# aouyang1/go-muse

Measured on AMD Instinct MI355X. Metric: series-pairs XCorr/sec at N=4096, 1M-series batch; achieved HBM GB/s, higher is better.
Workload: dtype f64

## Files before the change

### go-muse_amd/binding.py

```python
import ctypes
import os

import numpy as np

from . import build as _build

_i32 = ctypes.c_int32
_i64 = ctypes.c_int64
_f64 = ctypes.c_double
_vp = ctypes.c_void_p
_dp = ctypes.POINTER(ctypes.c_double)
_i32p = ctypes.POINTER(ctypes.c_int32)
_i64p = ctypes.POINTER(ctypes.c_int64)

MUSE_OK = 0
MUSE_ERR_INVALID = -1
MUSE_ERR_LENGTH = -2
MUSE_ERR_ZERO_STD = -3
MUSE_ERR_NO_DEVICE = -4
MUSE_ERR_HIP = -5
MUSE_ERR_UNSUPPORTED = -6
MUSE_ERR_NOMEM = -7
MUSE_ERR_EMPTY = -8
MUSE_LAG_WINDOW_MAX = 63
# ... 118 lines not shown
    "muse_batch_score_many_in_window": (ctypes.c_int, [ctypes.POINTER(_vp), _i32, _i32]),
    "muse_batch_run_many_in_window": (ctypes.c_int, [ctypes.POINTER(_vp), _i32, _i32p, _i32, _i32, _i32, _f64, _i32, _i32,
                                                     _i64p, _i32p, _dp, _i32p, _dp]),
    "muse_test_many_in_window_plan": (ctypes.c_int, [_i32, _i32, _i32, _i32, _i32p]),
    "muse_batch_score_many_in_lag_range": (ctypes.c_int, [ctypes.POINTER(_vp), _i32, _i32, _i32]),
    "muse_batch_run_many_in_lag_range": (ctypes.c_int, [ctypes.POINTER(_vp), _i32, _i32p, _i32, _i32, _i32, _i32, _f64, _i32, _i32,
                                                        _i64p, _i32p, _dp, _i32p, _dp]),
    "muse_test_many_lag_range_plan": (ctypes.c_int, [_i32, _i32, _i32, _i32, _i32, _i32p]),
    "muse_test_window_many_plan_rows": (ctypes.c_int, [_i32, _i32, _i32p, _i32p, _i32p, _i32p, _i32p, _i32p]),
    "muse_batch_run_many": (ctypes.c_int, [ctypes.POINTER(_vp), _i32, _i32p, _i32, _i32, _i32, _f64, _i32, _i32,
                                           _i64p, _i32p, _dp, _i32p, _dp]),
    "muse_batch_free": (ctypes.c_int, [_vp]),
    "muse_xcorr_with_x": (ctypes.c_int, [_vp, _dp, _dp, _i32, _i32, _dp, _i32p, _dp, _i32p]),
    "muse_xcorr": (ctypes.c_int, [_vp, _dp, _i32, _dp, _i32, _i32, _i32, _dp, _i32p, _dp, _i32p]),
    "muse_xcorr_groups": (ctypes.c_int, [_vp, _vp, _i32, _i32, _i32p, _dp, _i32p, _dp]),
    "muse_xcorr_batch": (ctypes.c_int, [_vp, _dp, _dp, _i64, _i32, _i32, _i32, _i32, _i32p, _dp, _i32p, _dp]),
    "muse_ctx_set_spectrum_cache": (ctypes.c_int, [_vp, _i32]),
    "muse_group_spectrum_cache": (ctypes.c_int, [_vp, _i64p, _i64p]),
    "muse_group_drop_spectrum_cache": (ctypes.c_int, [_vp]),
    "muse_test_spectrum_cache_limits": (ctypes.c_int, [_vp, _i64, _i64]),
    "muse_test_spectrum_cache_reader": (ctypes.c_int, [_vp, _i32]),
    "muse_test_spectrum_cache_policy": (ctypes.c_int, [_i64, _i32, _i32, _i32, _i64, _i64, _i64, _i32p, _i64p, _i64p]),
    "muse_test_batch_redo_pairs": (ctypes.c_int, [_vp, _i64p, _i64, _i64p]),
    "muse_next_pow2": (_i64, [_f64]),
}


class MuseError(RuntimeError):
    def __init__(self, status, message):
        super().__init__("muse_hip status %d: %s" % (status, message))
        self.status = status
        self.message = message


_lib = None


def lib_path():
    return _build.LIB


def load():
    global _lib
    if _lib is None:
        path = lib_path()
        if not os.path.exists(path):
# ... 36 lines not shown
```

### go-muse_amd/csrc/capi_batch.hip

```cpp
#include "capi_internal.h"
#include "xcorr_huge.h"

using namespace muse;


int ilog2(int64_t n)
{
    int l = 0;
    while (((int64_t)1 << l) < n)
        l++;
    return l;
}

int build_spectrum(muse_ctx *ctx, const double *ref_host, int N, int n, int normalize, double x_scale,
                          double xc_scale, double2 *X, double2 *xc, float2 *xcf, double *xs, int *zero_std)
{
    double *dref = nullptr;
    int *dstat = nullptr;
    double2 *dscr = nullptr;
    HIP_TRY(dmalloc(ctx, &dref, (size_t)N * sizeof(double)));
    hipError_t e = dmalloc(ctx, &dstat, sizeof(int));
    if (e == hipSuccess && n > GENERIC_LDS_MAX_N)
        e = dmalloc(ctx, &dscr, (size_t)n * sizeof(double2));
    if (e == hipSuccess)
// ... 518 lines not shown
    return MUSE_OK;
}

extern "C" int muse_test_batch_redo_pairs(muse_batch *b, int64_t *pairs, int64_t cap, int64_t *count)
{
    if (!b || !count || cap < 0 || (cap > 0 && !pairs))
        return fail(MUSE_ERR_INVALID, "bad redo-list arguments");
    *count = 0;
    int rc = use_device(b->ctx);
    if (rc)
        return rc;
    HIP_TRY(hipStreamSynchronize(b->stream()));
    if (!b->ovf_count || !b->ovf_list.p)
        return MUSE_OK;
    int listed = 0;
    HIP_TRY(hipMemcpy(&listed, b->ovf_count, sizeof(int), hipMemcpyDeviceToHost));
    *count = listed;
    const int64_t k = std::min<int64_t>(std::min<int64_t>(listed, cap), b->ovf_list.cap);
    if (k > 0)
        HIP_TRY(hipMemcpy(pairs, b->ovf_list.p, (size_t)k * sizeof(long long), hipMemcpyDeviceToHost));
    return MUSE_OK;
}

extern "C" int muse_batch_score(muse_batch *b)
{
    return batch_score(b, ScorePass{});
}

static int check_mask(const muse_batch *b, int variant, const LagRange &mask)
{
    if (!(variant == KERNEL_R16_FOLD || variant == KERNEL_R16_OCC3 || (variant == KERNEL_SMALL && b->logn <= 11)) || 2 * mask.hi > b->n)
        return fail(MUSE_ERR_UNSUPPORTED, "the masked transform pass runs on the default kernels of FFT lengths 512 ... 4096");
    if (2 * mask.lneg > b->n - 2)
        return fail(MUSE_ERR_UNSUPPORTED, "the masked transform pass takes at most n / 2 - 1 lags below zero");
    return MUSE_OK;
}

int batch_score_check(muse_batch *b, const LagRange *mask, int *variant)
{
    *variant = -1;
    if (b->n > GENERIC_MAX_N)
        return b->g->f32 ? fail(MUSE_ERR_UNSUPPORTED, "float32-storage groups run on the default kernels only (FFT lengths 512 ... 16384)") : MUSE_OK;
    const KernelChoice kc = choose_kernel(b, (b->g->M + 1) / 2);
    if (kc.error)
        return fail(MUSE_ERR_UNSUPPORTED, "%s", kc.error);
    if (mask && check_mask(b, kc.variant, *mask))
// ... 47 lines not shown
        rc = check_mask(b, variant, *mask);
        if (rc)
            return rc;
        b->origin = ScoreOrigin::in_window(MUSE_IN_WINDOW_MASKED, *mask, variant);
        set_window(p, *mask);
    }
    const bool allow_spectrum_cache = pass.allow_spectrum_cache;
    const SlideFuse *slide = pass.slide;
    if (slide) {
        if (variant != KERNEL_R16_FOLD || allow_spectrum_cache)
            return fail(MUSE_ERR_INVALID, "the fused slide runs in the default n = 4096 kernel, off the rows");
        p.slide_tails = slide->tails;
        p.slide_k = slide->k;
    }
    if (variant == KERNEL_GENERIC && b->n <= GENERIC_LDS_MAX_N)
        p.gscratch = nullptr;
    LaunchTimer timer(ctx, false, st);
    LaunchTimer redo_timer(ctx, true, st);
    if (variant == KERNEL_R16_FOLD) {
        HIP_TRY(b->ovf_list.ensure(ctx, 2 * p.npairs, st));
        p.ovf_count = b->ovf_count;
        p.work_counter = b->ovf_count + 1;
        p.ovf_list = b->ovf_list.p;
        HIP_TRY(hipMemsetAsync(b->ovf_count, 0, 2 * sizeof(int), st));
        ZcPlan plan;
        std::unique_lock<std::mutex> zc_lock(b->g->ready_mu, std::defer_lock);
        if (allow_spectrum_cache && !mask && spectrum_cache_candidate(b, variant)) {
            zc_lock.lock();
            rc = plan_spectrum_cache(b, plan);
            if (rc)
                return rc;
            if (!plan.use)
                zc_lock.unlock();
        }
        HIP_TRY(timer.begin());
        if (plan.use) {
            bool launched = false;
            const auto next_launch = [&]() {
                const hipError_t e = launched ? hipMemsetAsync(b->ovf_count + 1, 0, sizeof(int), st) : hipSuccess;
                launched = true;
                return e;
            };
            const bool occ4_reader = ctx->zc_reader.load() == 1;
            for (const auto &sg : plan.readers) {
                FusedParams r = p;
                r.npairs = sg.pairs;
                HIP_TRY(next_launch());
                HIP_TRY(launch_cached(r, SpectrumCacheArgs{sg.zc(), sg.zstat(), sg.pair0, sg.pairs}, ctx->num_cus, st, occ4_reader));
            }
            if (plan.tail_pair0 < p.npairs) {
                FusedParams w = p;
                w.npairs = p.npairs - plan.tail_pair0;
                HIP_TRY(next_launch());
                HIP_TRY(launch_cache_fill(w, SpectrumCacheArgs{plan.tail_zpairs ? plan.tail_seg.zc() : nullptr,
                                                               plan.tail_zpairs ? plan.tail_seg.zstat() : nullptr,
                                                               plan.tail_pair0, plan.tail_zpairs}, ctx->num_cus, st));
            }
            zc_lock.unlock();
        } else {
            HIP_TRY(launch_fused(p, variant, ctx->num_cus, st));
        }
        HIP_TRY(timer.end());
        FusedParams q = p;
        q.slide_tails = nullptr;
        q.slide_k = 0;
        q.pair_list = b->ovf_list.p;
        q.pair_count = b->ovf_count;
        q.dense_total = ctx->variant == 0 ? p.npairs : 0;
        q.npairs = std::min<long long>(p.npairs, (long long)ctx->num_cus * 3);
        HIP_TRY(redo_timer.begin());
        HIP_TRY(launch_fused(q, KERNEL_R16_OCC3, ctx->num_cus, st));
        HIP_TRY(redo_timer.end());
        if (p.npairs >= 1024 && !(b->handoff_host && b->handoff_M == M && b->handoff_rewrites == b->g->rewrites)) {
            if (!b->handoff_host)
                HIP_TRY(hmalloc(ctx, &b->handoff_host, sizeof(int)));
            *b->handoff_host = 0;
            b->handoff_M = M;
            b->handoff_rewrites = b->g->rewrites;
            HIP_TRY(hipMemcpyAsync(b->handoff_host, b->ovf_count, sizeof(int), hipMemcpyDeviceToHost, st));
        }
    } else if (variant == KERNEL_LONG) {
        HIP_TRY(b->ovf_list.ensure(ctx, 2 * p.npairs, st));
        p.ovf_count = b->ovf_count;
        p.ovf_list = b->ovf_list.p;
        HIP_TRY(hipMemsetAsync(b->ovf_count, 0, 2 * sizeof(int), st));
        HIP_TRY(timer.begin());
        HIP_TRY(launch_fused(p, variant, ctx->num_cus, st));
        HIP_TRY(timer.end());
        FusedParams q = p;
        q.pair_list = b->ovf_list.p;
        q.pair_count = b->ovf_count;
        q.npairs = std::min<long long>(p.npairs, (long long)ctx->num_cus * STOCKHAM_GLOBAL_WGS_PER_CU);
        HIP_TRY(redo_timer.begin());
        HIP_TRY(launch_fused(q, KERNEL_STOCKHAM, ctx->num_cus, st));
        HIP_TRY(redo_timer.end());
    } else {
        HIP_TRY(timer.begin());
        HIP_TRY(launch_fused(p, variant, ctx->num_cus, st));
        HIP_TRY(timer.end());
    }
    return MUSE_OK;
}

extern "C" int muse_batch_scores(muse_batch *b, int32_t *lag, double *mv)
{
    int rc = muse_batch_score(b);
    if (rc)
        return rc;
    const int64_t M = b->g->M;
    if (M == 0)
        return MUSE_OK;
    if (!lag || !mv)
        return fail(MUSE_ERR_INVALID, "NULL output");
    HIP_TRY(hipMemcpyAsync(lag, b->lag.p, (size_t)M * sizeof(int), hipMemcpyDeviceToHost, b->stream()));
    HIP_TRY(hipMemcpyAsync(mv, b->mv.p, (size_t)M * sizeof(double), hipMemcpyDeviceToHost, b->stream()));
    HIP_TRY(hipStreamSynchronize(b->stream()));
    return MUSE_OK;
}

extern "C" int muse_batch_kernel_name(muse_batch *b, char *name, int32_t cap)
{
    if (!b || !name || cap < 1)
        return fail(MUSE_ERR_INVALID, "NULL argument");
    char k[96] = "xcorr_fused_generic";
    const char *padded = b->N < b->n ? "true" : "false", *f32 = b->g->f32 ? "true" : "false";
    const ScoreOrigin &o = b->origin;
    if (o.slide == MUSE_SLIDE_IN_WINDOW_FUSED) {
        snprintf(k, sizeof(k), "xcorr_fused_n4096_fold<false, %s, %s, %s, true>", padded, f32, o.kind == ScoreOrigin::MASKED ? "true" : "false");
    } else if (o.kind == ScoreOrigin::MASKED) {
        if (o.variant == ScoreOrigin::MANY && b->n == 4096)
            snprintf(k, sizeof(k), "xcorr_fused_n4096_fold_multi<%s, %s, true>", padded, f32);
        else if (o.variant == ScoreOrigin::MANY)
            snprintf(k, sizeof(k), "xcorr_fused_small<%d, %s, true, false, true>", b->logn, padded);
        else if (b->n == 4096 && o.variant == KERNEL_R16_OCC3)
            snprintf(k, sizeof(k), "xcorr_fused_n4096_occ4<%s, 3, false, %s, true>", padded, f32);
        else if (b->n == 4096)
            snprintf(k, sizeof(k), "xcorr_fused_n4096_fold<false, %s, %s, true>", padded, f32);
        else
            snprintf(k, sizeof(k), "xcorr_fused_small<%d, %s, false, %s, true>", b->logn, padded, f32);
// ... 99 lines not shown
```

### go-muse_amd/csrc/capi_context.hip

```cpp
#include "capi_internal.h"

using namespace muse;


thread_local std::string g_last_error;

int fail(int status, const char *fmt, ...)
{
    char buf[512];
    va_list ap;
    va_start(ap, fmt);
    vsnprintf(buf, sizeof(buf), fmt, ap);
    va_end(ap);
    g_last_error = buf;
    return status;
}

extern "C" int muse_abi_version(void) { return MUSE_HIP_ABI_VERSION; }
extern "C" const char *muse_last_error(void) { return g_last_error.c_str(); }
extern "C" const char *muse_status_string(int s)
{
    switch (s) {
    case MUSE_OK: return "ok";
    case MUSE_ERR_INVALID: return "invalid argument";
// ... 286 lines not shown
                            fprintf(f, " %llu", h[((size_t)wg * 16 + w) * 16 + i]);
                        fprintf(f, "\n");
                    }
                fclose(f);
            }
        }
    }
#endif
    (void)hipFree(ctx->dbg_stamps);
    rows_slots_free(ctx);
    huge_free(ctx);
    ctx->gscratch.release(ctx);
    ctx->zscratch.release(ctx);
    ctx->many_tab.release(ctx);
    for (auto &p : ctx->small_free)
        (void)hipHostFree(p.first);
    ctx->small_free.clear();
    pool_drain(ctx);
    for (auto *ev : {&ctx->events, &ctx->redo_events})
        for (auto &e : *ev) {
            (void)hipEventDestroy(e.first);
            (void)hipEventDestroy(e.second);
        }
    (void)hipFree(ctx->tw1);
    (void)hipFree(ctx->tw2);
    (void)hipFree(ctx->twm);
    (void)hipFree(ctx->twmf);
    (void)hipFree(ctx->tw1f);
    (void)hipFree(ctx->g2);
    (void)hipFree(ctx->g3a);
    (void)hipFree(ctx->g3b);
    for (int k = 0; k < 5; k++)
        (void)hipFree(ctx->gsmall[k]);
    (void)hipFree(ctx->wsplit);
    for (int k = 0; k < 3; k++)
        (void)hipFree(ctx->twl[k]);
    for (double *b : ctx->stage_pool)
        (void)hipHostFree(b);
    (void)hipFree(ctx->tw2f);
    if (ctx->probe_stream) {
        if (ctx->probe_buf)
            *((volatile int *)(ctx->probe_buf + 2 * PROBE_WINDOWS) + 1) = 1;
        (void)hipStreamSynchronize(ctx->probe_stream);
        (void)hipStreamDestroy(ctx->probe_stream);
    }
    if (ctx->probe_buf)
// ... 11 lines not shown

extern "C" int muse_ctx_synchronize(muse_ctx *ctx)
{
    int rc = use_device(ctx);
    if (rc)
        return rc;
    HIP_TRY(hipStreamSynchronize(ctx->stream));
    return MUSE_OK;
}

extern "C" int muse_ctx_trim(muse_ctx *ctx)
{
    int rc = use_device(ctx);
    if (rc)
        return rc;
    pool_drain(ctx);
    std::vector<std::pair<unsigned char *, int>> slots;
    {
        std::lock_guard<std::mutex> lock(ctx->small_mu);
        slots.swap(ctx->small_free);
    }
    for (auto &p : slots)
        (void)hipHostFree(p.first);
    return MUSE_OK;
}

extern "C" int muse_test_pool_stats(muse_ctx *ctx, int64_t *dev_idle_bytes, int64_t *dev_idle_blocks, int64_t *host_idle_bytes,
                                    int64_t *host_idle_blocks)
{
    if (!ctx)
        return fail(MUSE_ERR_INVALID, "NULL context");
    {
        std::lock_guard<std::mutex> lock(ctx->dev_pool.mu);
        if (dev_idle_bytes)
            *dev_idle_bytes = (int64_t)ctx->dev_pool.idle_bytes;
        if (dev_idle_blocks)
            *dev_idle_blocks = (int64_t)ctx->dev_pool.idle.size();
    }
    {
        std::lock_guard<std::mutex> lock(ctx->host_pool.mu);
        if (host_idle_bytes)
            *host_idle_bytes = (int64_t)ctx->host_pool.idle_bytes;
        if (host_idle_blocks)
            *host_idle_blocks = (int64_t)ctx->host_pool.idle.size();
    }
    return MUSE_OK;
// ... 25 lines not shown
    if (!ctx || !(variant == 0 || variant == 1 || variant == 7 || variant == 10 || variant == 11 || variant == 12 || variant == 13 || variant == 14 || variant == 15))
        return fail(MUSE_ERR_INVALID, "bad kernel variant (0 auto, 1 generic, 7 rescaling n=4096, 10 default n=4096, 11 Stockham, 12 half-round, 13 long series, 14 real transform, 15 real transform on the 16 x 1024 split)");
    ctx->variant = variant;
    return MUSE_OK;
}

extern "C" int muse_ctx_set_screening(muse_ctx *ctx, int32_t enable)
{
    if (!ctx)
        return fail(MUSE_ERR_INVALID, "NULL context");
    ctx->screening = enable != 0;
    ctx->screen_min_rows = enable > 1 ? enable : 0;
    return MUSE_OK;
}

extern "C" int muse_ctx_kernel_timing(muse_ctx *ctx, int32_t enable)
{
    if (!ctx)
        return fail(MUSE_ERR_INVALID, "NULL context");
    ctx->timing = enable != 0;
    return MUSE_OK;
}

static int drain_events(std::vector<std::pair<hipEvent_t, hipEvent_t>> &ev, double &ms_sum, int64_t &count)
{
    for (auto &e : ev) {
        HIP_TRY(hipEventSynchronize(e.second));
        float ms = 0.f;
        HIP_TRY(hipEventElapsedTime(&ms, e.first, e.second));
        ms_sum += (double)ms;
        count += 1;
        (void)hipEventDestroy(e.first);
        (void)hipEventDestroy(e.second);
    }
    ev.clear();
    return MUSE_OK;
}

extern "C" int muse_ctx_kernel_time(muse_ctx *ctx, double *total_ms, int64_t *launches)
{
    int rc = use_device(ctx);
    if (rc)
        return rc;
    rc = drain_events(ctx->events, ctx->total_ms, ctx->launches);
    if (rc)
        return rc;
    if (total_ms)
        *total_ms = ctx->total_ms;
    if (launches)
        *launches = ctx->launches;
    ctx->total_ms = 0.0;
    ctx->launches = 0;
    return MUSE_OK;
}

extern "C" int muse_ctx_redo_time(muse_ctx *ctx, double *total_ms, int64_t *brackets)
{
    int rc = use_device(ctx);
    if (rc)
        return rc;
    rc = drain_events(ctx->redo_events, ctx->redo_ms, ctx->redo_launches);
    if (rc)
        return rc;
    if (total_ms)
        *total_ms = ctx->redo_ms;
    if (brackets)
        *brackets = ctx->redo_launches;
    ctx->redo_ms = 0.0;
    ctx->redo_launches = 0;
    return MUSE_OK;
}

extern "C" int muse_ctx_device_pci_bus_id(muse_ctx *ctx, char *out, int32_t cap)
{
    if (!ctx || !out || cap < 16)
        return fail(MUSE_ERR_INVALID, "muse_ctx_device_pci_bus_id: NULL argument or a buffer under 16 bytes");
    snprintf(out, (size_t)cap, "%s", ctx->pci);
    return MUSE_OK;
}

extern "C" int muse_test_clock_probe_stop(muse_ctx *ctx)
{
    if (!ctx)
        return fail(MUSE_ERR_INVALID, "NULL context");
// ... 72 lines not shown
```

### go-muse_amd/csrc/capi_internal.h

```cpp
#pragma once
#include <hip/hip_runtime.h>

#include <algorithm>
#include <atomic>
#include <mutex>
#include <cmath>
#include <cstdarg>
#include <cstdio>
#include <cstdlib>
#include <cstring>
#include <ctime>
#include <limits>
#include <map>
#include <new>
#include <string>
#include <unordered_map>
#include <utility>
#include <vector>

#include "muse_hip.h"
#include "muse_hip_test.h"
#include "xcorr_kernels.h"

using namespace muse;
// ... 35 lines not shown
        if (e == hipSuccess)
            cap = count;
        return e;
    }
    void release(muse_ctx *ctx)
    {
        pool_free(ctx, Host, p);
        p = nullptr;
        cap = 0;
    }
};
template <class T> using HostBuf = PoolBuf<T, true>;
struct HugeWork {
    double2 *thi[4] = {nullptr, nullptr, nullptr, nullptr}, *tlo[4] = {nullptr, nullptr, nullptr, nullptr};
    PoolBuf<double2> Y, T;
    PoolBuf<double> part, snorm, sfin, sfin_x, amax;
    PoolBuf<double2> Y2;
    PoolBuf<double> amax2;
    hipStream_t stream2 = nullptr;
    hipEvent_t fork = nullptr, join = nullptr;
};
constexpr int64_t ZC_MIN_ROWS = 65536;
constexpr int ZC_MAX_SEGMENTS = 64;
constexpr int PROBE_WINDOWS = 4096;
struct muse_ctx {
    int device = 0;
    hipStream_t stream = nullptr;
    hipStream_t copy_stream = nullptr;
    int num_cus = 0;
    int64_t hbm = 0;
    char name[64] = {0};
    double2 *tw1 = nullptr, *tw2 = nullptr, *twm = nullptr;
    double2 *g2 = nullptr, *g3a = nullptr, *g3b = nullptr;
    double2 *twl[3] = {nullptr, nullptr, nullptr};
    double2 *gsmall[5] = {nullptr, nullptr, nullptr, nullptr, nullptr};
    double2 *wsplit = nullptr;
    float2 *tw1f = nullptr, *tw2f = nullptr, *twmf = nullptr;
    PoolBuf<double2> gscratch;
    std::vector<double *> stage_pool;
    std::mutex stage_mu;
    PoolBuf<double2> zscratch;
    PoolBuf<void *> many_tab;
    std::vector<void *> many_host;
    double screen_delta = 1e-4;
    int screening = 0;
    int64_t screen_min_rows = 0;
    double screen_e_scale = 1.0;
    int variant = 0;
    int xcorr_repeat = 1;
    unsigned long long *dbg_stamps = nullptr;
    hipStream_t probe_stream = nullptr;
    unsigned long long *probe_buf = nullptr;
    bool timing = false;
    std::vector<std::pair<hipEvent_t, hipEvent_t>> events, redo_events;
    double total_ms = 0.0, redo_ms = 0.0;
    int64_t launches = 0, redo_launches = 0;
    char pci[32] = {0};
    MemPool dev_pool, host_pool;
    HugeWork huge;
    int huge_batch_mb = 0;
    std::mutex huge_mu;
    std::mutex small_mu;
    std::vector<std::pair<unsigned char *, int>> small_free;
    unsigned long long small_token = 0;
    std::mutex timing_mu;
    std::atomic<bool> rows_always_copy{false};
    std::vector<void *> rows_slots;
    std::mutex rows_mu;
    std::atomic<int> zc_mode{1};
    std::atomic<int64_t> zc_min_rows{ZC_MIN_ROWS};
    std::atomic<int64_t> zc_budget{-1};
    std::atomic<int> zc_reader{0};
    std::atomic<int> win_rows_slices{0};
    std::atomic<bool> in_window_force{false};
    std::atomic<int> slide_in_window_force{0};
    std::atomic<bool> gather_nt{false};
    std::atomic<int> refs{1};
// ... 25 lines not shown
    hipEvent_t uploaded = nullptr;
    bool upload_pending = false;
    std::mutex ready_mu;
    HostBuf<long long> gidx_host;
    PoolBuf<long long> gidx_dev;
    hipEvent_t gather_done = nullptr;
    HostBuf<unsigned char> slide_host;
    PoolBuf<unsigned char> slide_dev;
    hipEvent_t slide_copied[2] = {nullptr, nullptr};
    struct ZcSegment {
        void *mem = nullptr;
        int64_t pair0 = 0, pairs = 0;
        double2 *zc() const { return (double2 *)mem; }
        double *zstat() const { return (double *)((char *)mem + (size_t)pairs * 4096 * sizeof(double2)); }
    };
    enum { ZC_NONE = 0, ZC_DECLINED = 1, ZC_VALID = 2 };
    std::vector<ZcSegment> zc_segs;
    int zc_state = ZC_NONE;
    int64_t zc_rows = 0, zc_bytes = 0;
    uint64_t zc_rewrites = 0;
    int64_t zc_passes = 0;
    int64_t zc_declined_M = -1;
    bool transient = false;
};

inline std::atomic<uint64_t> g_spectrum_serial{0};
struct muse_spectrum {
    std::atomic<int> refs{1};
    const uint64_t serial = g_spectrum_serial.fetch_add(1, std::memory_order_relaxed) + 1;
    double2 *X = nullptr, *xc = nullptr, *xcp = nullptr;
    double2 *xcw = nullptr;
    float2 *xcf = nullptr;
    double *xs = nullptr;
    double *c1 = nullptr;
    double xmax = -1.0;
};

inline int window_lneg(int L, int n) { return 2 * L == n ? L - 1 : L; }
struct LagRange {
    int hi, lneg, origin;
    int rows() const { return origin + hi + 1; }
    bool every_lag(int64_t n) const { return 2 * (int64_t)hi == n && lneg == n / 2 - 1; }
};
inline LagRange lag_window_range(int64_t n, int64_t L)
{
    const int hi = (int)std::min<int64_t>(L, n / 2);
// ... 22 lines not shown
    static ScoreOrigin packed(int32_t tiles) { return ScoreOrigin{PACKED, LagRange{0, 0, 0}, 0, tiles}; }
    static ScoreOrigin in_window(int32_t path, const LagRange &w, int32_t variant = 0) { return ScoreOrigin{(Kind)path, w, variant}; }
    int32_t in_window_path() const { return kind > OWN ? (int32_t)kind : 0; }
    int32_t mfma_tiles() const { return (window.rows() + 15) / 16; }
};

struct muse_batch {
    muse_ctx *ctx = nullptr;
    muse_group *g = nullptr;
    hipStream_t own_stream = nullptr;
    hipStream_t stream() const { return own_stream ? own_stream : ctx->stream; }
    int32_t N = 0, n = 0, logn = 0;
    muse_spectrum *sp = nullptr;
    double *c1 = nullptr;
    double2 *X = nullptr, *xc = nullptr;
    double2 *xcp = nullptr;
    double2 *xcw = nullptr;
    float2 *xcf = nullptr;
    double *xs = nullptr;
    int *ovf_count = nullptr;
    int *handoff_host = nullptr;
    int64_t handoff_M = -1;
    uint64_t handoff_rewrites = 0;
    PoolBuf<long long> ovf_list;
    PoolBuf<double> mv;
    PoolBuf<int> lag;
    unsigned char *small_out = nullptr;
    int small_cap = 0;
    PoolBuf<int> gid_dev;
    std::vector<int32_t> gid_host;
    bool gid_valid = false;
    PoolBuf<unsigned long long> gkey;
    PoolBuf<long long> gfirst, gwin;
    GroupWork gw() const { return GroupWork{gkey.p, gfirst.p, gwin.p}; }
    PoolBuf<muse_record> rec;
    PoolBuf<unsigned long long> selkey;
    PoolBuf<muse_record> cand;
    PoolBuf<int> cnt;
    HostBuf<muse_record> cand_host;
    HostBuf<int> cnt_host;
    HostBuf<muse_record> rec_host;
    HostBuf<unsigned long long> key_host;
    PoolBuf<unsigned> scr_flags;
    PoolBuf<double> scr_var;
    PoolBuf<unsigned char> include;
    PoolBuf<unsigned long long> scr_keys;
// ... 21 lines not shown
    int64_t guard_trips = 0;
    uint64_t guard_salt = 0;
    int32_t lag_window = -1;
    int32_t win_key = -1;
    PoolBuf<double> win_e, win_pw;
    bool windowed() const { return lag_window >= 0; }
    ScoreOrigin origin;
};

int use_device(muse_ctx *ctx);

struct LaunchTimer {
    muse_ctx *ctx;
    hipEvent_t e0 = nullptr, e1 = nullptr;
    bool redo;
    hipStream_t stream;
    explicit LaunchTimer(muse_ctx *c, bool redo_ = false, hipStream_t s = nullptr) : ctx(c), redo(redo_), stream(s ? s : c->stream) {}
    LaunchTimer(const LaunchTimer &) = delete;
    LaunchTimer &operator=(const LaunchTimer &) = delete;
    hipError_t begin()
    {
        if (!ctx->timing)
            return hipSuccess;
        hipError_t e = hipEventCreate(&e0);
        if (e == hipSuccess)
            e = hipEventCreate(&e1);
        if (e == hipSuccess)
            e = hipEventRecord(e0, stream);
        return e;
    }
    hipError_t end()
    {
        if (!e0 || !e1)
            return hipSuccess;
        const hipError_t e = hipEventRecord(e1, stream);
        if (e == hipSuccess) {
            std::lock_guard<std::mutex> lock(ctx->timing_mu);
            (redo ? ctx->redo_events : ctx->events).emplace_back(e0, e1);
            e0 = e1 = nullptr;
        }
        return e;
    }
    ~LaunchTimer()
    {
        if (e0)
            (void)hipEventDestroy(e0);
        if (e1)
            (void)hipEventDestroy(e1);
// ... 24 lines not shown
void adopt_spectrum(muse_batch *b);
int build_spectrum(muse_ctx *ctx, const double *ref_host, int N, int n, int normalize, double x_scale,
                          double xc_scale, double2 *X, double2 *xc, float2 *xcf, double *xs, int *zero_std);
hipError_t ensure_gscratch(muse_ctx *ctx, int64_t n, int slices_per_cu = muse::GSCRATCH_SLICES_PER_CU);
hipError_t ensure_twl(muse_ctx *ctx, int64_t n);
int ensure_scores(muse_batch *b);
struct SlideFuse {
    const void *tails;
    int32_t k;
};
struct ScorePass {
    bool allow_spectrum_cache = true;
    const LagRange *window = nullptr;
    int32_t path = MUSE_IN_WINDOW_PLAIN;
    const SlideFuse *slide = nullptr;
    const LagRange *mask() const { return window && path == MUSE_IN_WINDOW_MASKED ? window : nullptr; }
    bool direct() const { return window && path == MUSE_IN_WINDOW_MFMA; }
};
int batch_score(muse_batch *b, const ScorePass &pass);
int batch_score_check(muse_batch *b, const LagRange *mask, int *variant);
enum { ZC_POLICY_NONE = 0, ZC_POLICY_BUILD = 1, ZC_POLICY_DECLINED = 2 };
int spectrum_cache_policy(int64_t rows, int32_t N, bool f32, int mode, int64_t min_rows, int64_t free_bytes, int64_t budget,
                          int64_t *rows_cached, int64_t *bytes);
void group_drop_spectrum_cache(muse_group *g);
int check_window_request(const muse_batch *b, int32_t max_lag, bool f32);
int window_tables(muse_batch *b, const LagRange &w, PoolBuf<double> &e, PoolBuf<double> &pw, int32_t *key, hipStream_t st);
muse::WindowParams window_params(const muse_batch *b, const LagRange &w, const double *e, const double *pw);
int score_direct(muse_batch *b, const LagRange &w, bool bracket = true);
int window_plan(int32_t N, bool f32, const LagRange &w, bool force_transform);
int plan_in_window(muse_batch *b, const LagRange &w, ScorePass *pass);
int score_in_window(muse_batch *b, const LagRange &w);
inline void set_window(muse::FusedParams &p, const LagRange &w)
{
    p.win = 1;
    p.win_lpos = w.hi;
    p.win_lneg = w.lneg;
}
int check_own_window(const muse_batch *b, int32_t lag_lo, int32_t lag_hi, int r = -1);
inline int32_t range_max_lag(int32_t lag_lo, int32_t lag_hi)
{
    return (int32_t)std::min<int64_t>(std::max<int64_t>(-(int64_t)lag_lo, lag_hi), INT32_MAX);
}
muse::FusedParams base_params(muse_batch *b);
int ensure_select_ws(muse_batch *b, int64_t M, int64_t G, bool with_gid, int K, bool on_device);
inline bool select_on_device(int32_t top_n, int64_t G) { return top_n <= TOPN_DEVICE_MAX && G > EXACT_FEED_MAX_GROUPS; }
muse_batch::RunKey run_key(const muse_batch *b, const int32_t *group_id, int64_t G, int32_t max_lag, int32_t top_n,
// ... 37 lines not shown
```

### go-muse_amd/csrc/capi_many.hip

```cpp
#include "capi_internal.h"

using namespace muse;


int upload_many_tab(muse_ctx *ctx, std::vector<void *> &tab, bool zscratch)
{
    if (zscratch)
        HIP_TRY(ctx->zscratch.ensure(ctx, (int64_t)ctx->num_cus * 4 * 4096, ctx->stream));
    HIP_TRY(ctx->many_tab.ensure(ctx, (int64_t)tab.size(), ctx->stream));
    HIP_TRY(hipStreamSynchronize(ctx->stream));
    ctx->many_host.swap(tab);
    HIP_TRY(hipMemcpyAsync(ctx->many_tab.p, ctx->many_host.data(), ctx->many_host.size() * sizeof(void *),
                           hipMemcpyHostToDevice, ctx->stream));
    return MUSE_OK;
}

extern "C" int muse_batch_read_scores(muse_batch *b, int32_t *lag, double *mv)
{
    if (!b)
        return fail(MUSE_ERR_INVALID, "NULL batch");
    int rc = use_device(b->ctx);
    if (rc)
        return rc;
    const int64_t M = b->g->M;
    if (M == 0)
        return MUSE_OK;
    if (!lag || !mv)
        return fail(MUSE_ERR_INVALID, "NULL output");
    if (M > b->mv.cap || M > b->lag.cap)
        return fail(MUSE_ERR_INVALID, "the batch has not been scored since the group grew");
    if (!b->scores_exact) {
        rc = muse_batch_score(b);
        if (rc)
            return rc;
    }
    HIP_TRY(hipMemcpyAsync(lag, b->lag.p, (size_t)M * sizeof(int), hipMemcpyDeviceToHost, b->ctx->stream));
    HIP_TRY(hipMemcpyAsync(mv, b->mv.p, (size_t)M * sizeof(double), hipMemcpyDeviceToHost, b->ctx->stream));
    HIP_TRY(hipStreamSynchronize(b->ctx->stream));
    return MUSE_OK;
}

int check_batch_list(muse_batch *const *bs, int32_t R)
{
    if (!bs || R < 1)
        return fail(MUSE_ERR_INVALID, "bad batch list");
    for (int r = 0; r < R; r++) {
        if (!bs[r])
            return fail(MUSE_ERR_INVALID, "NULL batch in list");
        if (bs[r]->ctx != bs[0]->ctx || bs[r]->g != bs[0]->g)
            return fail(MUSE_ERR_INVALID, "batches of one pass must share the context and the comparison group");
        for (int q = 0; q < r; q++)
            if (bs[q] == bs[r])
                return fail(MUSE_ERR_INVALID, "the same batch appears twice in the list");
    }
    return MUSE_OK;
}

ManyKind many_kind(muse_batch *const *bs, int32_t R)
{
    muse_batch *b0 = bs[0];
    muse_ctx *ctx = b0->ctx;
// ... 50 lines not shown
    void **const t = ctx->many_tab.p;
    FusedParams p = base_params(b0);
    p.R = R;
    p.xcp_many = (const double2 *const *)t;
    p.mv_many = (double *const *)(t + R);
    p.lag_many = (int *const *)(t + 2 * R);
    p.c1_many = (const double *const *)(t + 3 * R);
    p.zscratch = ctx->zscratch.p;
    p.zslots = (int)(ctx->zscratch.cap / 4096);
    if (mask)
        set_window(p, *mask);
    HIP_TRY(b0->ovf_list.ensure(ctx, 2 * p.npairs, b0->stream()));
    p.ovf_count = b0->ovf_count;
    p.work_counter = b0->ovf_count + 1;
    p.ovf_list = b0->ovf_list.p;
    std::unique_lock<std::mutex> scratch_lock(ctx->stage_mu, std::defer_lock);
    if (long_n || real_n) {
        scratch_lock.lock();
        p.gscratch = ctx->gscratch.p;
        p.gscratch_slices = (long long)(ctx->gscratch.cap / b0->n);
    }
    LaunchTimer timer(ctx);
    HIP_TRY(hipMemsetAsync(b0->ovf_count, 0, 2 * sizeof(int), ctx->stream));
    HIP_TRY(timer.begin());
    if (small_n) {
        HIP_TRY(launch_fused_small(p, ctx->num_cus, ctx->stream));
    } else if (real_n) {
        p.gsmall = ctx->gsmall[4];
        HIP_TRY(launch_fused_real_split(p, ctx->num_cus, ctx->stream));
    } else if (long_n)
        HIP_TRY(launch_fused_long(p, ctx->num_cus, ctx->stream));
    else
        HIP_TRY(launch_fused_multi(p, ctx->num_cus, ctx->stream));
    HIP_TRY(timer.end());
    const bool redo = !small_n && !real_n;
    LaunchTimer redo_timer(ctx, true);
    if (redo)
        HIP_TRY(redo_timer.begin());
    for (int r = 0; r < R && redo; r++) {
        FusedParams q = base_params(bs[r]);
        q.pair_list = b0->ovf_list.p;
        q.pair_count = b0->ovf_count;
        if (mask)
            set_window(q, *mask);
        if (long_n) {
            q.npairs = std::min<long long>(q.npairs, (long long)ctx->num_cus * STOCKHAM_GLOBAL_WGS_PER_CU);
// ... 80 lines not shown
```

### go-muse_amd/csrc/capi_rows.hip

```cpp
#include "capi_internal.h"

using namespace muse;

namespace {
constexpr size_t ROWS_GUARD = 8192;
constexpr size_t ROWS_SLOT_MIN_ELEMS = 1u << 16;
constexpr size_t ROWS_SLOT_MAX_ELEMS = 1u << 24;
constexpr size_t ROWS_ZERO_COPY_BYTES = 256u << 10;
constexpr size_t ROWS_SLOT_KEEP_ELEMS = 1u << 20;
constexpr int ROWS_SLOTS_KEPT = 16;
}

struct RowsSlot {
    muse_group g;
    muse_batch b;
    double *dev = nullptr;
    double *host = nullptr;
    double *host_dev = nullptr;
    size_t cap_elems = 0;
    SingleGroupOut *out = nullptr;
    hipEvent_t done = nullptr;
    hipStream_t stream = nullptr;
    PoolBuf<double> win_e, win_pw, win_slabs;
    uint64_t win_serial = 0;
// ... 143 lines not shown
    slot_destroy(s);
}

static int slot_take(muse_batch *tmpl, int64_t M, size_t elems, RowsSlot **out, bool windowed = false)
{
    muse_ctx *ctx = tmpl->ctx;
    const int32_t N = tmpl->N;
    RowsSlot *s = nullptr;
    int rc = slot_acquire(ctx, elems, &s);
    if (rc)
        return rc;
    s->g.N = N;
    s->g.stride = N;
    s->g.M = M;
    s->g.cap = M;
    s->g.hstats_rows = 0;
    s->g.transient = true;
    s->b.N = tmpl->N;
    s->b.n = tmpl->n;
    s->b.logn = tmpl->logn;
    s->b.sp = tmpl->sp;
    adopt_spectrum(&s->b);
    s->b.handoff_M = -1;
    s->b.own_stream = tmpl->n >= GENERIC_LDS_MAX_N && !windowed ? nullptr : s->stream;
    const int64_t cap = std::max<int64_t>(M, 4096);
    hipError_t ea = s->b.mv.ensure(ctx, cap, s->stream);
    if (ea == hipSuccess)
        ea = s->b.lag.ensure(ctx, cap, s->stream);
    if (ea != hipSuccess) {
        slot_destroy(s);
        return fail(MUSE_ERR_NOMEM, "hipMalloc failed: %s", hipGetErrorString(ea));
    }
    *out = s;
    return MUSE_OK;
}

static int rows_lag_range_plan(int64_t M, int32_t N, int num_cus, const LagRange &w, int *panels, int *S)
{
    const int64_t n = muse_next_pow2((double)N);
    *panels = 0;
    *S = 0;
    if (w.every_lag(n))
        return MUSE_ROWS_LAG_RANGE_PLAIN;
    if (n > GENERIC_MAX_N || w.rows() > WIN_PANEL_MAX_ROWS)
        return MUSE_ROWS_LAG_RANGE_UNSUPPORTED;
    if (w.rows() <= 2 * MUSE_LAG_WINDOW_MAX + 1) {
// ... 490 lines not shown
```

### go-muse_amd/csrc/capi_run.hip

```cpp
#include "capi_internal.h"

using namespace muse;


namespace {
struct GoHeap {
    std::vector<muse_record> h;
    static bool less(const muse_record &a, const muse_record &b) { return std::fabs(a.score) < std::fabs(b.score); }
    void up(size_t j)
    {
        for (;;) {
            if (j == 0)
                break;
            size_t i = (j - 1) / 2;
            if (!less(h[j], h[i]))
                break;
            std::swap(h[i], h[j]);
            j = i;
        }
    }
    void down(size_t i0, size_t n)
    {
        size_t i = i0;
        for (;;) {
// ... 282 lines not shown
        for (int64_t blk = 0; blk < nb; blk++)
            for (int r = 0; r < cnt[(size_t)blk]; r++)
                cands.push_back(cand[(size_t)(blk * K + r)]);
        if (screened && (int64_t)*b->refine_host * 4 > (M + 1) / 2)
            b->costly_key = rkey;
        if (screened && screen_guard_tripped(b))
            return run_select(b, group_id, G_in, series_offset, max_lag, top_n, threshold, sign_filter, abs_scores, out, false);
    } else {
        HIP_TRY(launch_group_reduce(sp, b->gw(), b->rec.p, b->selkey.p, b->stream()));
        const muse_record *rec = b->rec_host.p;
        const unsigned long long *key = b->key_host.p;
        HIP_TRY(hipMemcpyAsync(b->rec_host.p, b->rec.p, (size_t)G * sizeof(muse_record), hipMemcpyDeviceToHost, b->stream()));
        HIP_TRY(hipMemcpyAsync(b->key_host.p, b->selkey.p, (size_t)G * sizeof(unsigned long long), hipMemcpyDeviceToHost,
                               b->stream()));
        HIP_TRY(hipStreamSynchronize(b->stream()));
        for (int64_t g = 0; g < G; g++)
            if (key[(size_t)g] != 0ull)
                cands.push_back(rec[(size_t)g]);
        if (screened && (int64_t)*b->refine_host * 4 > (M + 1) / 2)
            b->costly_key = rkey;
        if (screened && screen_guard_tripped(b))
            return run_select(b, group_id, G_in, series_offset, max_lag, top_n, threshold, sign_filter, abs_scores, out, false);
    }
    if (!group_id)
        for (auto &r : cands)
            r.group = (int32_t)std::min<int64_t>(r.series, 0x7fffffffLL);
    out = heap_select(std::move(cands), top_n);
    return MUSE_OK;
}

void emit(const std::vector<muse_record> &sel, int64_t *out_series, int32_t *out_lag, double *out_score,
                 int32_t *out_count, double *out_mean_abs)
{
    double sum = 0.0;
    for (size_t i = sel.size(); i-- > 0;) {
        if (out_series)
            out_series[i] = sel[i].series;
        if (out_lag)
            out_lag[i] = sel[i].lag;
        if (out_score)
            out_score[i] = sel[i].score;
        sum += std::fabs(sel[i].score);
    }
    if (out_count)
        *out_count = (int32_t)sel.size();
    if (out_mean_abs)
// ... 180 lines not shown
```

### go-muse_amd/csrc/capi_screen.hip

```cpp
#include "capi_internal.h"

using namespace muse;


muse_batch::RunKey run_key(const muse_batch *b, const int32_t *group_id, int64_t G, int32_t max_lag, int32_t top_n,
                                  double threshold, int32_t sign_filter, int32_t abs_scores)
{
    muse_batch::RunKey k;
    k.M = b->g->M;
    k.G = group_id ? G : 0;
    k.grouped = group_id ? 1 : 0;
    k.max_lag = max_lag;
    k.top_n = top_n;
    k.threshold = threshold;
    k.sign_filter = sign_filter;
    k.abs_scores = abs_scores ? 1 : 0;
    return k;
}

int32_t screen_path(const muse_batch *b, const muse_batch::RunKey &key, bool already_scored)
{
    const muse_ctx *ctx = b->ctx;
    const int64_t M = b->g->M;
    const bool length_ok = b->n >= 512 && b->n <= 65536;
// ... 55 lines not shown
    HIP_TRY(b->scr_keys.ensure(ctx, nkeys, st));
    if (!b->refine_host)
        HIP_TRY(hmalloc(b->ctx, &b->refine_host, sizeof(int)));
    if (!b->err_host)
        HIP_TRY(hmalloc(b->ctx, &b->err_host, sizeof(unsigned long long)));
    if (!b->err_dev)
        HIP_TRY(dmalloc(b->ctx, &b->err_dev, sizeof(unsigned long long)));
    HIP_TRY(b->est_save.ensure(ctx, 4 * npairs, st));
    HIP_TRY(b->ovf_list.ensure(ctx, 2 * npairs, st));
    if (b->sp->xmax < 0.0) {
        std::vector<double2> X((size_t)(b->n / 2 + 1));
        HIP_TRY(hipMemcpyAsync(X.data(), b->X, X.size() * sizeof(double2), hipMemcpyDeviceToHost, ctx->stream));
        HIP_TRY(hipStreamSynchronize(ctx->stream));
        double m = 0.0;
        for (const double2 &x : X)
            m = std::max(m, std::hypot(x.x, x.y));
        b->sp->xmax = m;
    }
    plan.Es = screen_error_scaled(b->sp->xmax, b->n) * ctx->screen_e_scale;
    HIP_TRY(hipMemsetAsync(b->err_dev, 0, sizeof(unsigned long long), ctx->stream));
    HIP_TRY(hipMemsetAsync(b->scr_flags.p, 0, (size_t)M * sizeof(unsigned), ctx->stream));
    HIP_TRY(hipMemsetAsync(b->include.p, 0, (size_t)M, ctx->stream));
    HIP_TRY(hipMemsetAsync(b->ovf_count, 0, 2 * sizeof(int), ctx->stream));
    return MUSE_OK;
}

static FusedParams screen_pass_params(muse_batch *b, int32_t max_lag, const ScreenPlan &plan, bool need_sign = true)
{
    FusedParams p = base_params(b);
    p.scr_need_sign = need_sign ? 1 : 0;
    p.scr_flags = b->scr_flags.p;
    p.scr_var = b->scr_var.p;
    p.scr_max_lag = max_lag;
    p.screen_delta = 2.0 * plan.Es;
    return p;
}

static int screen_finish(muse_batch *b, int32_t top_n, double threshold, int32_t sign_filter, int32_t abs_scores,
                         const int *gid_dev, int64_t G, const ScreenPlan &plan)
{
    muse_ctx *ctx = b->ctx;
    const int64_t M = b->g->M;
    const int64_t npairs = (M + 1) / 2;
    const double Es = plan.Es;
    ScreenSelect q{};
    q.mv = b->mv.p;
// ... 214 lines not shown
```

### go-muse_amd/csrc/reduce_kernels.hip

```cpp
#include <hip/hip_runtime.h>
#include <stdint.h>

#include "xcorr_kernels.h"

namespace muse {

constexpr long long IDX_NONE = 0x7fffffffffffffffLL;

__device__ __forceinline__ double clamp_score(double mv, int abs_scores)
{
    if (abs_scores) {
        double v = fabs(mv);
        if (v > 1.0)
            v = 1.0;
        return v;
    }
    double v = mv;
    if (v > 1.0)
        v = 1.0;
    else if (v < -1.0)
        v = -1.0;
    return v;
}
__device__ __forceinline__ unsigned long long abs_bits(double v)
// ... 275 lines not shown
        ci = wave_min_i32(ci);
        if (lane == 0)
            si[wave] = ci;
        __syncthreads();
        const int CI = min(min(si[0], si[1]), min(si[2], si[3]));
        if (t == (CI & 255)) {
            const int mm = CI >> 8;
#pragma unroll
            for (int m = 0; m < 16; m++)
                if (m == mm)
                    k[m] = 0ull;
            cand[(long long)blockIdx.x * K + r] = rec[base + CI];
        }
        __syncthreads();
    }
    if (t == 0)
        cnt[blockIdx.x] = r;
}


__global__ __launch_bounds__(256) void topn_ungrouped_kernel(SelectParams sp, int K, SmallSlot *cand, CountSlot *cnt,
                                                             unsigned long long token)
{
    __shared__ unsigned long long sk[4];
    __shared__ int si[4];
    __shared__ int picked[TOPN_DEVICE_MAX];
    const int t = threadIdx.x, lane = t & 63, wave = t >> 6;
    const long long base = (long long)blockIdx.x * TOPN_CHUNK;
    unsigned long long k[16];
#pragma unroll
    for (int m = 0; m < 16; m++) {
        const long long g = base + t + 256 * m;
        k[m] = 0ull;
        if (g < sp.G) {
            const double s = clamp_score(sp.mv[g], sp.abs_scores);
            if (passed(s, sp.lag[g], sp))
                k[m] = abs_bits(s) + 1ull;
        }
    }
    int r = 0;
    for (; r < K; r++) {
        unsigned long long bk = 0ull;
        int bm = 0;
#pragma unroll
        for (int m = 0; m < 16; m++)
            if (k[m] > bk) {
                bk = k[m];
                bm = m;
            }
        const unsigned long long wk = wave_max_u64(bk);
        if (lane == 0)
            sk[wave] = wk;
        __syncthreads();
        unsigned long long BK = sk[0];
        BK = sk[1] > BK ? sk[1] : BK;
        BK = sk[2] > BK ? sk[2] : BK;
        BK = sk[3] > BK ? sk[3] : BK;
        if (BK == 0ull)
            break;
        int ci = (bk == BK) ? (t + 256 * bm) : 0x7fffffff;
        ci = wave_min_i32(ci);
        if (lane == 0)
            si[wave] = ci;
        __syncthreads();
        const int CI = min(min(si[0], si[1]), min(si[2], si[3]));
        if (t == (CI & 255)) {
            const int mm = CI >> 8;
#pragma unroll
            for (int m = 0; m < 16; m++)
                if (m == mm)
                    k[m] = 0ull;
            picked[r] = CI;
        }
        __syncthreads();
    }
    __syncthreads();
    for (int i = t; i < r; i += 256) {
        const long long g = base + picked[i];
        muse_record rec;
        rec.series = g + sp.series_offset;
        rec.score = clamp_score(sp.mv[g], sp.abs_scores);
        rec.lag = sp.lag[g];
        rec.group = 0;
        write_slot(cand + (long long)blockIdx.x * K + i, rec, 1ull, token);
    }
    if (t == 0) {
        cnt[blockIdx.x].count = (unsigned long long)r;
        asm volatile("s_waitcnt vmcnt(0)" ::: "memory");
        cnt[blockIdx.x].stamp = token;
        asm volatile("" ::: "memory");
    }
}

hipError_t launch_topn_ungrouped(const SelectParams &sp, int K, SmallSlot *cand, CountSlot *cnt, unsigned long long token,
                                 hipStream_t stream)
{
    if (sp.G <= 0 || sp.group_id || sp.include || K < 1 || K > TOPN_DEVICE_MAX)
// ... 424 lines not shown
```

Before: 166.3 million.

## Skip redundant redo pass, pool timing events, and cut topn barriers

Records the overflow count from a previous full pass and skips the OCC3 redo launch when the same batch and rewrites produced zero overflows. It also avoids a redundant counter memset when the counters are known clean. Timing events are recycled from a pool instead of being created and destroyed on every launch. The top-n selection kernel now double-buffers its shared slots so each iteration needs one barrier instead of three. The risk is stale skip state if the invalidation of the cached redo count misses a path.

```diff
diff --git a/go-muse_amd/binding.py b/go-muse_amd/binding.py
--- a/go-muse_amd/binding.py
+++ b/go-muse_amd/binding.py
@@ -164,6 +164,8 @@
     "muse_test_spectrum_cache_reader": (ctypes.c_int, [_vp, _i32]),
     "muse_test_spectrum_cache_policy": (ctypes.c_int, [_i64, _i32, _i32, _i32, _i64, _i64, _i64, _i32p, _i64p, _i64p]),
     "muse_test_batch_redo_pairs": (ctypes.c_int, [_vp, _i64p, _i64, _i64p]),
+    "muse_test_event_pool": (ctypes.c_int, [_vp, _i64p]),
+    "muse_test_redo_skip_decision":(ctypes.c_int, [_i64, ctypes.c_uint64, _i64, _i64, ctypes.c_uint64, _i32, _i32p]),
     "muse_next_pow2": (_i64, [_f64]),
 }
 
diff --git a/go-muse_amd/csrc/capi_batch.hip b/go-muse_amd/csrc/capi_batch.hip
--- a/go-muse_amd/csrc/capi_batch.hip
+++ b/go-muse_amd/csrc/capi_batch.hip
@@ -564,6 +564,29 @@
     return MUSE_OK;
 }
 
+void publish_redo_count(muse_batch *b)
+{
+    if (!b->handoff_pending || !b->handoff_host)
+        return;
+    const int listed = *(volatile int *)b->handoff_host;
+    if (listed == HANDOFF_NONE)
+        return;
+    b->handoff_pending = false;
+    std::lock_guard<std::mutex> lock(b->g->ready_mu);
+    b->g->redo_M = b->handoff_M;
+    b->g->redo_rewrites = b->handoff_rewrites;
+    b->g->redo_count = listed;
+}
+
+extern "C" int muse_test_redo_skip_decision(int64_t known_M, uint64_t known_rewrites, int64_t known_count, int64_t M,
+                                            uint64_t rewrites, int32_t pass_kind, int32_t *skip)
+{
+    if (!skip)
+        return fail(MUSE_ERR_INVALID, "NULL output");
+    *skip = redo_skip_decision(known_M, known_rewrites, known_count, M, rewrites, pass_kind) ? 1 : 0;
+    return MUSE_OK;
+}
+
 extern "C" int muse_batch_score(muse_batch *b)
 {
     return batch_score(b, ScorePass{});
@@ -657,7 +680,15 @@
         p.ovf_count = b->ovf_count;
         p.work_counter = b->ovf_count + 1;
         p.ovf_list = b->ovf_list.p;
-        HIP_TRY(hipMemsetAsync(b->ovf_count, 0, 2 * sizeof(int), st));
+        bool skip_redo = false;
+        {
+            std::lock_guard<std::mutex> lock(b->g->ready_mu);
+            skip_redo = redo_skip_decision(b->g->redo_M, b->g->redo_rewrites, b->g->redo_count, M, b->g->rewrites,
+                                           slide ? REDO_PASS_SLIDE : mask ? REDO_PASS_MASKED : REDO_PASS_FULL);
+        }
+        if (!(b->counters_clean && b->clean_stream == st))
+            HIP_TRY(hipMemsetAsync(b->ovf_count, 0, 2 * sizeof(int), st));
+        b->counters_clean = false;
         ZcPlan plan;
         std::unique_lock<std::mutex> zc_lock(b->g->ready_mu, std::defer_lock);
         if (allow_spectrum_cache && !mask && spectrum_cache_candidate(b, variant)) {
@@ -703,22 +734,31 @@
         q.pair_count = b->ovf_count;
         q.dense_total = ctx->variant == 0 ? p.npairs : 0;
         q.npairs = std::min<long long>(p.npairs, (long long)ctx->num_cus * 3);
-        HIP_TRY(redo_timer.begin());
-        HIP_TRY(launch_fused(q, KERNEL_R16_OCC3, ctx->num_cus, st));
-        HIP_TRY(redo_timer.end());
+        if (!skip_redo) {
+            HIP_TRY(redo_timer.begin());
+            HIP_TRY(launch_fused(q, KERNEL_R16_OCC3, ctx->num_cus, st));
+            HIP_TRY(redo_timer.end());
+        }
         if (p.npairs >= 1024 && !(b->handoff_host && b->handoff_M == M && b->handoff_rewrites == b->g->rewrites)) {
             if (!b->handoff_host)
                 HIP_TRY(hmalloc(ctx, &b->handoff_host, sizeof(int)));
-            *b->handoff_host = 0;
+            *b->handoff_host = HANDOFF_NONE;
             b->handoff_M = M;
             b->handoff_rewrites = b->g->rewrites;
+            b->handoff_pending = !slide && !b->g->transient;
             HIP_TRY(hipMemcpyAsync(b->handoff_host, b->ovf_count, sizeof(int), hipMemcpyDeviceToHost, st));
+        }
+        if (skip_redo) {
+            HIP_TRY(hipMemsetAsync(b->ovf_count + 1, 0, sizeof(int), st));
+            b->counters_clean = true;
+            b->clean_stream = st;
         }
     } else if (variant == KERNEL_LONG) {
         HIP_TRY(b->ovf_list.ensure(ctx, 2 * p.npairs, st));
         p.ovf_count = b->ovf_count;
         p.ovf_list = b->ovf_list.p;
         HIP_TRY(hipMemsetAsync(b->ovf_count, 0, 2 * sizeof(int), st));
+        b->counters_clean = false;
         HIP_TRY(timer.begin());
         HIP_TRY(launch_fused(p, variant, ctx->num_cus, st));
         HIP_TRY(timer.end());
@@ -750,6 +790,7 @@
     HIP_TRY(hipMemcpyAsync(lag, b->lag.p, (size_t)M * sizeof(int), hipMemcpyDeviceToHost, b->stream()));
     HIP_TRY(hipMemcpyAsync(mv, b->mv.p, (size_t)M * sizeof(double), hipMemcpyDeviceToHost, b->stream()));
     HIP_TRY(hipStreamSynchronize(b->stream()));
+    publish_redo_count(b);
     return MUSE_OK;
 }
 
diff --git a/go-muse_amd/csrc/capi_context.hip b/go-muse_amd/csrc/capi_context.hip
--- a/go-muse_amd/csrc/capi_context.hip
+++ b/go-muse_amd/csrc/capi_context.hip
@@ -332,6 +332,8 @@
             (void)hipEventDestroy(e.first);
             (void)hipEventDestroy(e.second);
         }
+    for (hipEvent_t e : ctx->event_pool)
+        (void)hipEventDestroy(e);
     (void)hipFree(ctx->tw1);
     (void)hipFree(ctx->tw2);
     (void)hipFree(ctx->twm);
@@ -389,6 +391,22 @@
     }
     for (auto &p : slots)
         (void)hipHostFree(p.first);
+    std::vector<hipEvent_t> idle;
+    {
+        std::lock_guard<std::mutex> lock(ctx->timing_mu);
+        idle.swap(ctx->event_pool);
+    }
+    for (hipEvent_t e : idle)
+        (void)hipEventDestroy(e);
+    return MUSE_OK;
+}
+
+extern "C" int muse_test_event_pool(muse_ctx *ctx, int64_t *idle_events)
+{
+    if (!ctx || !idle_events)
+        return fail(MUSE_ERR_INVALID, "NULL argument");
+    std::lock_guard<std::mutex> lock(ctx->timing_mu);
+    *idle_events = (int64_t)ctx->event_pool.size();
     return MUSE_OK;
 }
 
@@ -460,7 +478,7 @@
     return MUSE_OK;
 }
 
-static int drain_events(std::vector<std::pair<hipEvent_t, hipEvent_t>> &ev, double &ms_sum, int64_t &count)
+static int drain_events(muse_ctx *ctx, std::vector<std::pair<hipEvent_t, hipEvent_t>> &ev, double &ms_sum, int64_t &count)
 {
     for (auto &e : ev) {
         HIP_TRY(hipEventSynchronize(e.second));
@@ -468,9 +486,15 @@
         HIP_TRY(hipEventElapsedTime(&ms, e.first, e.second));
         ms_sum += (double)ms;
         count += 1;
-        (void)hipEventDestroy(e.first);
-        (void)hipEventDestroy(e.second);
-    }
+    }
+    std::lock_guard<std::mutex> lock(ctx->timing_mu);
+    for (auto &e : ev)
+        for (hipEvent_t one : {e.first, e.second}) {
+            if (ctx->event_pool.size() < EVENT_POOL_MAX)
+                ctx->event_pool.push_back(one);
+            else
+                (void)hipEventDestroy(one);
+        }
     ev.clear();
     return MUSE_OK;
 }
@@ -480,7 +504,7 @@
     int rc = use_device(ctx);
     if (rc)
         return rc;
-    rc = drain_events(ctx->events, ctx->total_ms, ctx->launches);
+    rc = drain_events(ctx, ctx->events, ctx->total_ms, ctx->launches);
     if (rc)
         return rc;
     if (total_ms)
@@ -497,7 +521,7 @@
     int rc = use_device(ctx);
     if (rc)
         return rc;
-    rc = drain_events(ctx->redo_events, ctx->redo_ms, ctx->redo_launches);
+    rc = drain_events(ctx, ctx->redo_events, ctx->redo_ms, ctx->redo_launches);
     if (rc)
         return rc;
     if (total_ms)
diff --git a/go-muse_amd/csrc/capi_internal.h b/go-muse_amd/csrc/capi_internal.h
--- a/go-muse_amd/csrc/capi_internal.h
+++ b/go-muse_amd/csrc/capi_internal.h
@@ -81,6 +81,7 @@
 };
 constexpr int64_t ZC_MIN_ROWS = 65536;
 constexpr int ZC_MAX_SEGMENTS = 64;
+constexpr size_t EVENT_POOL_MAX = 64;
 constexpr int PROBE_WINDOWS = 4096;
 struct muse_ctx {
     int device = 0;
@@ -112,6 +113,7 @@
     unsigned long long *probe_buf = nullptr;
     bool timing = false;
     std::vector<std::pair<hipEvent_t, hipEvent_t>> events, redo_events;
+    std::vector<hipEvent_t> event_pool;
     double total_ms = 0.0, redo_ms = 0.0;
     int64_t launches = 0, redo_launches = 0;
     char pci[32] = {0};
@@ -183,6 +185,9 @@
     int64_t zc_passes = 0;
     int64_t zc_declined_M = -1;
     bool transient = false;
+    int64_t redo_M = -1;
+    uint64_t redo_rewrites = 0;
+    int64_t redo_count = 0;
 };
 
 inline std::atomic<uint64_t> g_spectrum_serial{0};
@@ -251,6 +256,9 @@
     int *handoff_host = nullptr;
     int64_t handoff_M = -1;
     uint64_t handoff_rewrites = 0;
+    bool handoff_pending = false;
+    bool counters_clean = false;
+    hipStream_t clean_stream = nullptr;
     PoolBuf<long long> ovf_list;
     PoolBuf<double> mv;
     PoolBuf<int> lag;
@@ -318,8 +326,16 @@
     {
         if (!ctx->timing)
             return hipSuccess;
-        hipError_t e = hipEventCreate(&e0);
-        if (e == hipSuccess)
+        {
+            std::lock_guard<std::mutex> lock(ctx->timing_mu);
+            for (hipEvent_t *ev : {&e0, &e1})
+                if (!ctx->event_pool.empty()) {
+                    *ev = ctx->event_pool.back();
+                    ctx->event_pool.pop_back();
+                }
+        }
+        hipError_t e = e0 ? hipSuccess : hipEventCreate(&e0);
+        if (e == hipSuccess && !e1)
             e = hipEventCreate(&e1);
         if (e == hipSuccess)
             e = hipEventRecord(e0, stream);
@@ -390,6 +406,14 @@
 enum { ZC_POLICY_NONE = 0, ZC_POLICY_BUILD = 1, ZC_POLICY_DECLINED = 2 };
 int spectrum_cache_policy(int64_t rows, int32_t N, bool f32, int mode, int64_t min_rows, int64_t free_bytes, int64_t budget,
                           int64_t *rows_cached, int64_t *bytes);
+enum { REDO_PASS_FULL = 0, REDO_PASS_MASKED = 1, REDO_PASS_SLIDE = 2, REDO_PASS_PARTIAL = 3 };
+constexpr int HANDOFF_NONE = -1;
+inline bool redo_skip_decision(int64_t known_M, uint64_t known_rewrites, int64_t known_count, int64_t M, uint64_t rewrites, int pass_kind)
+{
+    return (pass_kind == REDO_PASS_FULL || pass_kind == REDO_PASS_MASKED) && M > 0 && known_M == M && known_rewrites == rewrites &&
+           known_count == 0;
+}
+void publish_redo_count(muse_batch *b);
 void group_drop_spectrum_cache(muse_group *g);
 int check_window_request(const muse_batch *b, int32_t max_lag, bool f32);
 int window_tables(muse_batch *b, const LagRange &w, PoolBuf<double> &e, PoolBuf<double> &pw, int32_t *key, hipStream_t st);
diff --git a/go-muse_amd/csrc/capi_many.hip b/go-muse_amd/csrc/capi_many.hip
--- a/go-muse_amd/csrc/capi_many.hip
+++ b/go-muse_amd/csrc/capi_many.hip
@@ -37,6 +37,8 @@
     HIP_TRY(hipMemcpyAsync(lag, b->lag.p, (size_t)M * sizeof(int), hipMemcpyDeviceToHost, b->ctx->stream));
     HIP_TRY(hipMemcpyAsync(mv, b->mv.p, (size_t)M * sizeof(double), hipMemcpyDeviceToHost, b->ctx->stream));
     HIP_TRY(hipStreamSynchronize(b->ctx->stream));
+    if (b->stream() == b->ctx->stream)
+        publish_redo_count(b);
     return MUSE_OK;
 }
 
@@ -133,6 +135,7 @@
     }
     LaunchTimer timer(ctx);
     HIP_TRY(hipMemsetAsync(b0->ovf_count, 0, 2 * sizeof(int), ctx->stream));
+    b0->counters_clean = false;
     HIP_TRY(timer.begin());
     if (small_n) {
         HIP_TRY(launch_fused_small(p, ctx->num_cus, ctx->stream));
diff --git a/go-muse_amd/csrc/capi_rows.hip b/go-muse_amd/csrc/capi_rows.hip
--- a/go-muse_amd/csrc/capi_rows.hip
+++ b/go-muse_amd/csrc/capi_rows.hip
@@ -189,6 +189,9 @@
     s->b.sp = tmpl->sp;
     adopt_spectrum(&s->b);
     s->b.handoff_M = -1;
+    s->b.handoff_pending = false;
+    s->g.redo_M = -1;
+    s->b.counters_clean = false;
     s->b.own_stream = tmpl->n >= GENERIC_LDS_MAX_N && !windowed ? nullptr : s->stream;
     const int64_t cap = std::max<int64_t>(M, 4096);
     hipError_t ea = s->b.mv.ensure(ctx, cap, s->stream);
diff --git a/go-muse_amd/csrc/capi_run.hip b/go-muse_amd/csrc/capi_run.hip
--- a/go-muse_amd/csrc/capi_run.hip
+++ b/go-muse_amd/csrc/capi_run.hip
@@ -328,6 +328,7 @@
         if (screened && screen_guard_tripped(b))
             return run_select(b, group_id, G_in, series_offset, max_lag, top_n, threshold, sign_filter, abs_scores, out, false);
     }
+    publish_redo_count(b);
     if (!group_id)
         for (auto &r : cands)
             r.group = (int32_t)std::min<int64_t>(r.series, 0x7fffffffLL);
diff --git a/go-muse_amd/csrc/capi_screen.hip b/go-muse_amd/csrc/capi_screen.hip
--- a/go-muse_amd/csrc/capi_screen.hip
+++ b/go-muse_amd/csrc/capi_screen.hip
@@ -101,6 +101,7 @@
     HIP_TRY(hipMemsetAsync(b->scr_flags.p, 0, (size_t)M * sizeof(unsigned), ctx->stream));
     HIP_TRY(hipMemsetAsync(b->include.p, 0, (size_t)M, ctx->stream));
     HIP_TRY(hipMemsetAsync(b->ovf_count, 0, 2 * sizeof(int), ctx->stream));
+    b->counters_clean = false;
     return MUSE_OK;
 }
 
diff --git a/go-muse_amd/csrc/reduce_kernels.hip b/go-muse_amd/csrc/reduce_kernels.hip
--- a/go-muse_amd/csrc/reduce_kernels.hip
+++ b/go-muse_amd/csrc/reduce_kernels.hip
@@ -321,8 +321,8 @@
 __global__ __launch_bounds__(256) void topn_ungrouped_kernel(SelectParams sp, int K, SmallSlot *cand, CountSlot *cnt,
                                                              unsigned long long token)
 {
-    __shared__ unsigned long long sk[4];
-    __shared__ int si[4];
+    __shared__ unsigned long long sk[2][4];
+    __shared__ int si[2][4];
     __shared__ int picked[TOPN_DEVICE_MAX];
     const int t = threadIdx.x, lane = t & 63, wave = t >> 6;
     const long long base = (long long)blockIdx.x * TOPN_CHUNK;
@@ -348,21 +348,26 @@
                 bm = m;
             }
         const unsigned long long wk = wave_max_u64(bk);
-        if (lane == 0)
-            sk[wave] = wk;
-        __syncthreads();
-        unsigned long long BK = sk[0];
-        BK = sk[1] > BK ? sk[1] : BK;
-        BK = sk[2] > BK ? sk[2] : BK;
-        BK = sk[3] > BK ? sk[3] : BK;
+        const int wi = wave_min_i32(bk == wk ? t + 256 * bm : 0x7fffffff);
+        const int buf = r & 1;
+        if (lane == 0) {
+            sk[buf][wave] = wk;
+            si[buf][wave] = wi;
+        }
+        __syncthreads();
+        unsigned long long BK = sk[buf][0];
+        int CI = si[buf][0];
+#pragma unroll
+        for (int w = 1; w < 4; w++) {
+            const unsigned long long kw = sk[buf][w];
+            const int iw = si[buf][w];
+            if (kw > BK || (kw == BK && iw < CI)) {
+                BK = kw;
+                CI = iw;
+            }
+        }
         if (BK == 0ull)
             break;
-        int ci = (bk == BK) ? (t + 256 * bm) : 0x7fffffff;
-        ci = wave_min_i32(ci);
-        if (lane == 0)
-            si[wave] = ci;
-        __syncthreads();
-        const int CI = min(min(si[0], si[1]), min(si[2], si[3]));
         if (t == (CI & 255)) {
             const int mm = CI >> 8;
 #pragma unroll
@@ -371,7 +376,6 @@
                     k[m] = 0ull;
             picked[r] = CI;
         }
-        __syncthreads();
     }
     __syncthreads();
     for (int i = t; i < r; i += 256) {
```

Result: no change. 166.6 million (median of 6 runs) (+0.2%).
